# kazuto1011/dusty-gan

Hardware: NVIDIA B200
Metric: chamfer_pairs_per_s (higher is better)
Workload: dtype f32

## Files before the change

dusty-gan_b200/csrc/chamfer.cu:

```cuda
#include <algorithm>

#include "common.cuh"

namespace dusty {
namespace chamfer {

constexpr int TPB = 256;
constexpr int TILE = 2048;
constexpr int CHUNK = 32;

struct Params {
  const float4* scanX;
  const float4* scanY;
  long long strideX, strideY;
  int countX, countY;
  int paddedX, paddedY;
  int row_begin, row_stride;
  int symmetric, mirror, compact_rows;
  float* M;
  long long ldm;
  float* dist1; float* dist2;
  int* idx1; int* idx2;
  const int2* metaX; const int2* metaY;
  const float4* boxX; const float4* boxY;
  const float4* bbX; const float4* bbY;
  const int* permX; const int* permY;
  unsigned long long* visited;
  unsigned long long* keys;
  int n_total, n_ref, offX, offY;
};

template <int NT>
__device__ __forceinline__ double block_sum(double v, double* red) {
  #pragma unroll
  for (int o = 16; o > 0; o >>= 1) v += __shfl_down_sync(0xffffffffu, v, o);
  const int warp = threadIdx.x >> 5, lane = threadIdx.x & 31;
  __syncthreads();
  if (lane == 0) red[warp] = v;
  __syncthreads();
  double s = 0.0;
  if (threadIdx.x == 0) {
    #pragma unroll
    for (int w = 0; w < NT / 32; ++w) s += red[w];
  }
  return s;
}

__device__ __forceinline__ float search_window(float ax, float ay, float az, float cur) {
  const float an = fmaf(az, az, fmaf(ax, ax, ay * ay));
  return fmaf(2.86102295e-6f , an + fmaxf(cur + an, 0.0f), 1e-36f);
}

template <bool WANT_INDEX>
__device__ __forceinline__ void warp_tile_exact_min(const float4* tp, int npairs, float ax, float ay, float az, int lane,
                                                    float& best, int& best_pos) {
  const f32x2 ax2 = pack2(ax, ax), ay2 = pack2(ay, ay), az2 = pack2(az, az);
  float e = __int_as_float(0x7f800000);
  int ei = 0x7fffffff;
  for (int q = lane; q < npairs; q += 32) {
    const float4 q0 = tp[2 * q], q1 = tp[2 * q + 1];
    const f32x2 dx = sub2(pack2(q0.x, q0.y), ax2);
    const f32x2 dy = sub2(pack2(q0.z, q0.w), ay2);
    const f32x2 dz = sub2(pack2(q1.x, q1.y), az2);
    float lo, hi;
    unpack2(fma2(dz, dz, fma2(dx, dx, mul2(dy, dy))), lo, hi);
    if (WANT_INDEX) {
      if (lo < e) { e = lo; ei = 2 * q; }
      if (hi < e) { e = hi; ei = 2 * q + 1; }
    } else {
      e = min3(e, lo, hi);
    }
  }
  float m = e;
  #pragma unroll
  for (int o = 16; o > 0; o >>= 1) m = fminf(m, __shfl_xor_sync(0xffffffffu, m, o));
  best = m;
  if (WANT_INDEX) {
    const bool mine = e == m && ei != 0x7fffffff;
    const unsigned key = mine ? (unsigned)ei : 0x7fffffffu;
    const unsigned kmin = __reduce_min_sync(0xffffffffu, key);
    const unsigned who = __ballot_sync(0xffffffffu, mine && key == kmin);
    best_pos = who ? __shfl_sync(0xffffffffu, ei, __ffs(who) - 1) : 0x7fffffff;
  }
}

template <bool WANT_INDEX>
__device__ __forceinline__ void warp_cloud_exact_min(const float4* cloud, int nchunks, const float4* boxes, float thr,
                                                     float ax, float ay, float az, int lane, const int* perm, float& best,
                                                     int& best_pos) {
  const f32x2 ax2 = pack2(ax, ax), ay2 = pack2(ay, ay), az2 = pack2(az, az);
  float e = __int_as_float(0x7f800000);
  int ei = 0x7fffffff;
  for (int ch = lane; ch < nchunks; ch += 32) {
    if (boxes != nullptr) {
      const float4 bl = boxes[2 * ch], bh = boxes[2 * ch + 1];
      const float gx = max3(0.0f, bl.x - ax, ax - bh.x), gy = max3(0.0f, bl.y - ay, ay - bh.y), gz = max3(0.0f, bl.z - az, az - bh.z);
      if (bl.w == 0.0f && fmaf(gz, gz, fmaf(gx, gx, __fmul_rn(gy, gy))) > thr) continue;
    }
    const float4* cp = cloud + (long long)ch * CHUNK;
    #pragma unroll 4
    for (int k = 0; k < CHUNK / 2; ++k) {
      const float4 q0 = cp[2 * k], q1 = cp[2 * k + 1];
      const f32x2 dx = sub2(pack2(q0.x, q0.y), ax2);
      const f32x2 dy = sub2(pack2(q0.z, q0.w), ay2);
      const f32x2 dz = sub2(pack2(q1.x, q1.y), az2);
      float lo, hi;
      unpack2(fma2(dz, dz, fma2(dx, dx, mul2(dy, dy))), lo, hi);
      if (WANT_INDEX) {
        const int i0 = ch * CHUNK + 2 * k;
        if (lo < e || (lo == e && ei != 0x7fffffff && (perm ? perm[i0] < perm[ei] : i0 < ei))) { e = lo; ei = i0; }
        if (hi < e || (hi == e && ei != 0x7fffffff && (perm ? perm[i0 + 1] < perm[ei] : i0 + 1 < ei))) { e = hi; ei = i0 + 1; }
      } else {
        e = min3(e, lo, hi);
      }
    }
  }
  float m = e;
  #pragma unroll
  for (int o = 16; o > 0; o >>= 1) m = fminf(m, __shfl_xor_sync(0xffffffffu, m, o));
  best = m;
  if (WANT_INDEX) {
    const bool mine = e == m && ei != 0x7fffffff;
    const unsigned key = mine ? (unsigned)(perm ? perm[ei] : ei) : 0x7fffffffu;
    const unsigned kmin = __reduce_min_sync(0xffffffffu, key);
    const unsigned who = __ballot_sync(0xffffffffu, mine && key == kmin);
    best_pos = who ? __shfl_sync(0xffffffffu, ei, __ffs(who) - 1) : 0x7fffffff;
  }
}

__device__ __forceinline__ void emit_entry(const Params& p, int ci, int cj, double S0, double S1) {
  const float v = (float)(S0 / (double)p.countX) + (float)(S1 / (double)p.countY);
  if (p.M) {
    p.M[(long long)(p.compact_rows ? (int)blockIdx.y : ci) * p.ldm + cj] = v;
    if (p.symmetric && p.mirror && ci != cj) p.M[(long long)cj * p.ldm + ci] = v;
  }
  if (p.keys) {
    const int gi = p.offX + ci, gj = p.offY + cj;
    if (gi != gj) {
      const unsigned long long vb = (unsigned long long)__float_as_uint(v) << 32;
      atomicMin(p.keys + gj, vb | (unsigned)gi);
      atomicMin(p.keys + gi, vb | (unsigned)gj);
      const int lo = min(gi, gj), hi = max(gi, gj);
      if (lo < p.n_ref && hi >= p.n_ref) {
        atomicMin(p.keys + p.n_total + hi, vb | (unsigned)lo);
        atomicMin(p.keys + 2 * (long long)p.n_total + lo, vb | (unsigned)hi);
      }
    }
  }
}

template <int R, bool MATRIX, bool MERGED, int NT = TPB>
__global__ void __launch_bounds__(NT, R >= 8 ? 512 / NT : (R == 4 ? 3 : 4)) nn_kernel(const Params p) {
  static_assert(!MERGED || MATRIX, "merged origins are a matrix front end layout");
  extern __shared__ __align__(128) unsigned char smem_raw[];
  float4* const tiles = reinterpret_cast<float4*>(smem_raw);
  __shared__ uint64_t bars[2];
  __shared__ double red[NT / 32];

  constexpr int RB = NT * R;
  constexpr int CH = (NT < TPB && !MERGED) ? CHUNK / 2 : CHUNK;
  constexpr int PR = CH / 2;
  const int tid = threadIdx.x;
  const int lane = tid & 31;

  int ci, cj;
  int dir_only = -1, rb_only = 0;
  if (MATRIX) {
    ci = p.row_begin + blockIdx.y * p.row_stride;
    cj = blockIdx.x;
    if (p.symmetric && cj < ci) return;
  } else {
    ci = cj = blockIdx.y;
    dir_only = blockIdx.z;
    rb_only = blockIdx.x;
    const int rows_here = dir_only == 0 ? p.countX : p.countY;
    if (rb_only >= (rows_here + RB - 1) / RB) return;
  }
  const float4* const sx = p.scanX + (long long)ci * p.strideX;
  const float4* const sy = p.scanY + (long long)cj * p.strideY;

  int2 mx = make_int2(p.countX, 1), my = make_int2(p.countY, 1);
  if (MERGED) { mx = p.metaX[ci]; my = p.metaY[cj]; }
#define K_ROW(r) (MERGED ? rb * RB + (tid >> 5) * (32 * R) + (r) * 32 + lane : rb * RB + (r) * NT + tid)
#define K_countX (MERGED ? mx.x : p.countX)
#define K_countY (MERGED ? my.x : p.countY)
#define K_paddedX (MERGED ? (mx.x + CHUNK - 1) / CHUNK * CHUNK : p.paddedX)
#define K_paddedY (MERGED ? (my.x + CHUNK - 1) / CHUNK * CHUNK : p.paddedY)

  const int ntX = (K_paddedX + TILE - 1) / TILE, ntY = (K_paddedY + TILE - 1) / TILE;
  const int nrbX = (K_countX + RB - 1) / RB, nrbY = (K_countY + RB - 1) / RB;
  const int seg0 = nrbX * ntY;
  int pos_begin, pos_end;
  if (MATRIX) { pos_begin = 0; pos_end = seg0 + nrbY * ntX; }
  else if (dir_only == 0) { pos_begin = rb_only * ntY; pos_end = pos_begin + ntY; }
  else { pos_begin = seg0 + rb_only * ntX; pos_end = pos_begin + ntX; }

  const int tstride = (R >= 8 && NT == TPB) ? TILE : min(TILE, max(p.paddedX, p.paddedY));
  if (tid == 0) { mbar_init(&bars[0], 1); mbar_init(&bars[1], 1); mbar_fence_init(); }
  __syncthreads();

  auto issue = [&](int pos, int buf) {
    int dir, t;
    if (pos < seg0) { dir = 0; t = pos % ntY; } else { dir = 1; t = (pos - seg0) % ntX; }
    const float4* src = (dir == 0 ? sy : sx) + (long long)t * TILE;
    const int padded = dir == 0 ? K_paddedY : K_paddedX;
    const int npts = min(TILE, padded - t * TILE);
    mbar_expect_tx(&bars[buf], (uint32_t)npts * 16u);
    bulk_g2s(tiles + buf * tstride, src, (uint32_t)npts * 16u, &bars[buf]);
  };
  if (tid == 0) issue(pos_begin, 0);

  f32x2 nax[R], nay[R], naz[R];
  float eb[R];
  int ei[R];
  float cur[R], sec[R];
  int cid[R];
// ... 128 lines not shown
        while (flagged) {
          const int src = __ffs(flagged) - 1;
          flagged &= flagged - 1;
          float m;
          int mi = 0;
          warp_tile_exact_min<!MATRIX>(tp, nch * PR, __shfl_sync(0xffffffffu, ax, src), __shfl_sync(0xffffffffu, ay, src),
                                       __shfl_sync(0xffffffffu, az, src), lane, m, mi);
          if (lane == src) {
            if (MATRIX) {
              eb[r] = fminf(eb[r], m);
            } else if (mi != 0x7fffffff) {
              mi += t * TILE;
              if (m < eb[r] || (m == eb[r] && mi < ei[r])) { eb[r] = m; ei[r] = mi; }
            }
          }
        }
      }
    }

    }

    if (MERGED && t == nt - 1 && rb * RB + (tid >> 5) * (32 * R) < rowcount) {
      const float4* const cand = dir == 0 ? sy : sx;
      #pragma unroll
      for (int r = 0; r < R; ++r) {
        float ax, ay, az, dummy;
        unpack2(nax[r], ax, dummy); unpack2(nay[r], ay, dummy); unpack2(naz[r], az, dummy);
        ax *= -0.5f; ay *= -0.5f; az *= -0.5f;
        const bool live = K_ROW(r) < rowcount;
        float e = __int_as_float(0x7f800000);
        if (live && cur[r] < __int_as_float(0x7f800000)) {
          const f32x2 ax2 = pack2(ax, ax), ay2 = pack2(ay, ay), az2 = pack2(az, az);
          const float4* cp = cand + (long long)cid[r] * CHUNK;
          #pragma unroll 4
          for (int k = 0; k < CHUNK / 2; ++k) {
            const float4 q0 = cp[2 * k], q1 = cp[2 * k + 1];
            const f32x2 dx = sub2(pack2(q0.x, q0.y), ax2);
            const f32x2 dy = sub2(pack2(q0.z, q0.w), ay2);
            const f32x2 dz = sub2(pack2(q1.x, q1.y), az2);
            float lo, hi;
            unpack2(fma2(dz, dz, fma2(dx, dx, mul2(dy, dy))), lo, hi);
            e = min3(e, lo, hi);
          }
        }
        eb[r] = e;
        const bool near_tie = live && sec[r] <= cur[r] + search_window(ax, ay, az, cur[r]);
        unsigned flagged = __ballot_sync(0xffffffffu, near_tie);
        while (flagged) {
          const int src = __ffs(flagged) - 1;
          flagged &= flagged - 1;
          float m;
          int mi;
          warp_cloud_exact_min<false>(cand, scanpadded / CHUNK, nullptr, 0.0f, __shfl_sync(0xffffffffu, ax, src),
                                      __shfl_sync(0xffffffffu, ay, src), __shfl_sync(0xffffffffu, az, src), lane, nullptr, m, mi);
          if (lane == src) eb[r] = fminf(eb[r], m);
        }
      }
    }

    if (t == nt - 1) {
      #pragma unroll
      for (int r = 0; r < R; ++r) {
        const int row = K_ROW(r);
        if (row < rowcount) {
          if (MATRIX) {
            if (MERGED) dsum += (row == rowcount - 1 ? (double)(dir == 0 ? mx.y : my.y) : 1.0) * (double)eb[r];
            else dsum += (double)eb[r];
          } else {
            float* dist = dir == 0 ? p.dist1 : p.dist2;
            int* idx = dir == 0 ? p.idx1 : p.idx2;
            const long long o = (long long)ci * rowcount + row;
            dist[o] = eb[r];
            if (idx) idx[o] = ei[r] == 0x7fffffff ? 0 : ei[r];
          }
        }
      }
    }
    if (MATRIX && pos == seg0 - 1) { S0 = block_sum<NT>(dsum, red); dsum = 0.0; }
    __syncthreads();
  }

  if (MATRIX) {
    const double S1 = block_sum<NT>(dsum, red);
    if (tid == 0) emit_entry(p, ci, cj, S0, S1);
  }
}

#undef K_ROW
#undef K_countX
#undef K_countY
#undef K_paddedX
#undef K_paddedY

__global__ void __launch_bounds__(256) prep_kernel(const float* __restrict__ xyz, long long clouds, int count,
                                                   int padded, float4* __restrict__ out) {
  const long long half = padded / 2;
  const long long g = (long long)blockIdx.x * blockDim.x + threadIdx.x;
  if (g >= clouds * half) return;
  const long long c = g / half;
  const int q = (int)(g - c * half);
  const float nan = __int_as_float(0x7fc00000);
  float v[2][4];
  #pragma unroll
  for (int s = 0; s < 2; ++s) {
    const int pt = 2 * q + s;
    if (pt < count) {
      const float* src = xyz + (c * count + pt) * 3;
      const float x = src[0], y = src[1], z = src[2];
      v[s][0] = x; v[s][1] = y; v[s][2] = z;
      v[s][3] = fmaf(z, z, fmaf(x, x, y * y));
    } else {
      v[s][0] = v[s][1] = v[s][2] = v[s][3] = nan;
    }
  }
  out[g * 2] = make_float4(v[0][0], v[1][0], v[0][1], v[1][1]);
  out[g * 2 + 1] = make_float4(v[0][2], v[1][2], v[0][3], v[1][3]);
}

__global__ void __launch_bounds__(256) prep_merge_kernel(const float* __restrict__ xyz, int count, long long stride,
                                                         float4* __restrict__ out, int2* __restrict__ meta) {
  __shared__ int wsum[8];
  const long long c = blockIdx.x;
  const int tid = threadIdx.x, lane = tid & 31, warp = tid >> 5;
  const float* src = xyz + c * count * 3;
  float* dst = reinterpret_cast<float*>(out + c * stride);
  const int per = (count + 255) / 256;
  const int begin = min(tid * per, count), end = min(begin + per, count);
  int mine = 0;
  for (int i = begin; i < end; ++i) mine += (src[3 * i] != 0.0f) || (src[3 * i + 1] != 0.0f) || (src[3 * i + 2] != 0.0f);
  int inc = mine;
  #pragma unroll
  for (int o = 1; o < 32; o <<= 1) { const int t = __shfl_up_sync(0xffffffffu, inc, o); if (lane >= o) inc += t; }
  if (lane == 31) wsum[warp] = inc;
  __syncthreads();
  int before = 0, total = 0;
  #pragma unroll
  for (int w = 0; w < 8; ++w) { if (w < warp) before += wsum[w]; total += wsum[w]; }
  auto put = [&](int pos, float x, float y, float z, float n) {
    float* q = dst + (size_t)(pos >> 1) * 8 + (pos & 1);
    q[0] = x; q[2] = y; q[4] = z; q[6] = n;
  };
  int pos = before + inc - mine;
  for (int i = begin; i < end; ++i) {
    const float x = src[3 * i], y = src[3 * i + 1], z = src[3 * i + 2];
    if (x != 0.0f || y != 0.0f || z != 0.0f) put(pos++, x, y, z, fmaf(z, z, fmaf(x, x, y * y)));
  }
  const int zeros = count - total;
  const int kept = total + (zeros > 0 ? 1 : 0);
  if (tid == 0) {
    if (zeros > 0) put(total, 0.0f, 0.0f, 0.0f, 0.0f);
    meta[c] = make_int2(kept, zeros > 0 ? zeros : 1);
  }
  const float nan = __int_as_float(0x7fc00000);
  const int padded = (kept + CHUNK - 1) / CHUNK * CHUNK;
  for (int i = kept + tid; i < padded; i += 256) put(i, nan, nan, nan, nan);
}

constexpr int SORT_CAP = 32768;
constexpr int SORT_TPB = 1024;
constexpr int WALK_BLOCKS = SORT_CAP / CHUNK / 32;

__device__ __forceinline__ unsigned spread7(unsigned v) {
  v &= 0x7fu;
  v = (v | (v << 4)) & 0x070fu;
  v = (v | (v << 2)) & 0x1333u;
  v = (v | (v << 1)) & 0x1555u;
  return v;
// ... 505 lines not shown
  if (n == 0 || m == 0) {
    if (n) DUSTY_CUDA(cudaMemsetAsync(grad_xyz1, 0, sizeof(float) * 3 * b * n, st));
    if (m) DUSTY_CUDA(cudaMemsetAsync(grad_xyz2, 0, sizeof(float) * 3 * b * m, st));
    return 0;
  }
  if (!xyz1 || !xyz2 || !grad_dist1 || !grad_dist2 || !idx1 || !idx2 || !grad_xyz1 || !grad_xyz2)
    return fail_arg(DUSTY_EINVAL, "chamfer_backward: null pointer");
  const GradArgs a{b, n, m, xyz1, xyz2, grad_dist1, grad_dist2, idx1, idx2, grad_xyz1, grad_xyz2};
  const long long total = (long long)b * n + (long long)b * m;
  const unsigned grid = (unsigned)((total + 255) / 256);
  grad_own_kernel<<<grid, 256, 0, st>>>(a);
  DUSTY_AFTER_LAUNCH("chamfer grad_own_kernel");
  grad_scatter_kernel<<<grid, 256, 0, st>>>(a);
  DUSTY_AFTER_LAUNCH("chamfer grad_scatter_kernel");
  return 0;
}

extern "C" size_t dusty_chamfer_matrix_workspace_bytes(int na, int pa, int nb, int pb) {
  size_t s = 0;
  if (na > 0 && pa > 0) s += align_up(scan_bytes(na, pa), 256) + meta_bytes(na) + box_bytes(na, pa);
  if (nb > 0 && pb > 0) s += align_up(scan_bytes(nb, pb), 256) + meta_bytes(nb) + box_bytes(nb, pb);
  return s;
}

namespace {
struct FusedKeys {
  unsigned long long* keys = nullptr;
  int n_total = 0, n_ref = 0, off_a = 0, off_b = 0;
};
}

static int matrix_impl(const float* A, int na, int pa, const float* B, int nb, int pb, int row_begin, int row_end,
                       int row_stride, int flags, float* M, long long ldm, const FusedKeys& fk, void* workspace,
                       size_t workspace_bytes, void* stream) {
  cudaStream_t st = static_cast<cudaStream_t>(stream);
  const int symmetric = (flags & DUSTY_MATRIX_SYMMETRIC) != 0, mirror = (flags & DUSTY_MATRIX_MIRROR) != 0;
  const int compact_rows = (flags & DUSTY_MATRIX_COMPACT_ROWS) != 0, prepared = (flags & DUSTY_MATRIX_PREPARED) != 0;
  const int merge = (flags & DUSTY_MATRIX_MERGE_ORIGIN) != 0;
  if (mirror && (!symmetric || compact_rows)) return fail_arg(DUSTY_EINVAL, "chamfer_matrix: MIRROR needs SYMMETRIC and excludes COMPACT_ROWS");
  if (na < 0 || nb < 0 || pa <= 0 || pb <= 0) return fail_arg(DUSTY_EINVAL, "chamfer_matrix: bad sizes na=%d pa=%d nb=%d pb=%d", na, pa, nb, pb);
  if (symmetric && (nb != na || pb != pa)) return fail_arg(DUSTY_EINVAL, "chamfer_matrix: symmetric needs nb==na and pb==pa");
  if (row_stride <= 0 || row_begin < 0 || row_end > na || (M && ldm < nb))
    return fail_arg(DUSTY_EINVAL, "chamfer_matrix: bad row range [%d,%d) stride %d of %d, ldm %lld", row_begin, row_end, row_stride, na, ldm);
  if (fk.keys && (fk.n_ref < 0 || fk.off_a < 0 || fk.off_b < 0 || fk.off_a + na > fk.n_total || fk.off_b + nb > fk.n_total ||
                  (symmetric && fk.off_a != fk.off_b)))
    return fail_arg(DUSTY_EINVAL, "chamfer_matrix_fused: offsets %d+%d, %d+%d do not fit %d stacked clouds", fk.off_a, na, fk.off_b, nb, fk.n_total);
  if (row_begin >= row_end || nb == 0) return 0;
  if (int rc = check_device()) return rc;
  if (!A || !B || (!M && !fk.keys) || !workspace) return fail_arg(DUSTY_EINVAL, "chamfer_matrix: null pointer");
  if (!aligned16(workspace)) return fail_arg(DUSTY_EALIGN, "chamfer_matrix: workspace must be 16-byte aligned");
  const size_t need = dusty_chamfer_matrix_workspace_bytes(na, pa, symmetric ? 0 : nb, pb);
  if (workspace_bytes < need) return fail_arg(DUSTY_ENOSPACE, "chamfer_matrix: workspace %zu < %zu", workspace_bytes, need);
  char* const wsp = static_cast<char*>(workspace);
  float4* sa = reinterpret_cast<float4*>(wsp);
  int2* ma = reinterpret_cast<int2*>(wsp + align_up(scan_bytes(na, pa), 256));
  float4* ba = reinterpret_cast<float4*>(wsp + align_up(scan_bytes(na, pa), 256) + meta_bytes(na));
  char* const wsb = wsp + align_up(scan_bytes(na, pa), 256) + meta_bytes(na) + box_bytes(na, pa);
  float4* sb = symmetric ? sa : reinterpret_cast<float4*>(wsb);
  int2* mb = symmetric ? ma : reinterpret_cast<int2*>(wsb + align_up(scan_bytes(nb, pb), 256));
  float4* bb = symmetric ? ba : reinterpret_cast<float4*>(wsb + align_up(scan_bytes(nb, pb), 256) + meta_bytes(nb));
  const bool pair = merge && pa <= PAIR_CAP && pb <= PAIR_CAP;
  const bool walk = merge && !pair && pa <= SORT_CAP && pb <= SORT_CAP;
  const bool sorted = pair || walk;
  if (!prepared) {
    if (sorted) {
      if (int rc = run_prep_sort2(sort_side(A, na, pa, sa, ma, ba, nullptr, nullptr), na,
                                  sort_side(B, nb, pb, sb, mb, bb, nullptr, nullptr), symmetric ? 0 : nb, st, true)) return rc;
    } else if (merge) {
      if (int rc = run_prep_merge(A, na, pa, sa, ma, st)) return rc;
      if (!symmetric) if (int rc = run_prep_merge(B, nb, pb, sb, mb, st)) return rc;
    } else {
      if (int rc = run_prep(A, na, pa, sa, st)) return rc;
      if (!symmetric) if (int rc = run_prep(B, nb, pb, sb, st)) return rc;
    }
  }
  const int rows = (row_end - row_begin + row_stride - 1) / row_stride;
  if (rows > 65535) return fail_arg(DUSTY_EINVAL, "chamfer_matrix: %d rows in one call exceeds 65535", rows);
  Params p{};
  p.scanX = sa; p.scanY = sb;
  p.countX = pa; p.countY = pb;
  p.paddedX = padded_of(pa); p.paddedY = padded_of(pb);
  p.strideX = p.paddedX; p.strideY = p.paddedY;
  p.row_begin = row_begin; p.row_stride = row_stride;
  p.symmetric = symmetric; p.mirror = mirror; p.compact_rows = compact_rows;
  p.M = M; p.ldm = ldm;
  p.keys = fk.keys; p.n_total = fk.n_total; p.n_ref = fk.n_ref; p.offX = fk.off_a; p.offY = fk.off_b;
  p.visited = g_visited_counter;
  const dim3 grid(nb, rows, 1);
  if (merge) {
    p.metaX = ma; p.metaY = mb;
    if (sorted) { p.boxX = ba; p.boxY = bb; p.bbX = block_boxes_of(ba, na, pa); p.bbY = symmetric ? p.bbX : block_boxes_of(bb, nb, pb); }
    if (pair) return launch_pair_split(p, grid, st);
    if (walk) return launch_walk_split<true>(p, grid, st);
    return launch_nn<8, true, true>(p, grid, st);
  }
  return dispatch_matrix(pa > pb ? pa : pb, p, grid, st);
}

extern "C" int dusty_chamfer_matrix(const float* A, int na, int pa, const float* B, int nb, int pb, int row_begin,
                                    int row_end, int row_stride, int flags, float* M, long long ldm, void* workspace,
                                    size_t workspace_bytes, void* stream) {
  if (!M) return fail_arg(DUSTY_EINVAL, "chamfer_matrix: null pointer");
  return matrix_impl(A, na, pa, B, nb, pb, row_begin, row_end, row_stride, flags, M, ldm, FusedKeys{}, workspace,
                     workspace_bytes, stream);
}

extern "C" size_t dusty_nn_keys_bytes(int n_total) { return n_total > 0 ? (size_t)3 * n_total * sizeof(unsigned long long) : 0; }

extern "C" int dusty_nn_keys_reset(uint64_t* keys, int n_total, void* stream) {
  if (n_total <= 0) return 0;
  if (!keys) return fail_arg(DUSTY_EINVAL, "nn_keys_reset: null pointer");
  DUSTY_CUDA(cudaMemsetAsync(keys, 0xff, dusty_nn_keys_bytes(n_total), static_cast<cudaStream_t>(stream)));
  return 0;
}

extern "C" int dusty_chamfer_matrix_fused(const float* A, int na, int pa, const float* B, int nb, int pb, int row_begin,
                                          int row_end, int row_stride, int flags, float* M, long long ldm, int stacked_offset_a,
                                          int stacked_offset_b, int n_ref, int n_total, uint64_t* keys, void* workspace,
                                          size_t workspace_bytes, void* stream) {
  if (!keys) return fail_arg(DUSTY_EINVAL, "chamfer_matrix_fused: null keys");
  FusedKeys fk;
  fk.keys = reinterpret_cast<unsigned long long*>(keys);
  fk.n_total = n_total; fk.n_ref = n_ref; fk.off_a = stacked_offset_a; fk.off_b = stacked_offset_b;
  return matrix_impl(A, na, pa, B, nb, pb, row_begin, row_end, row_stride, flags, M, ldm, fk, workspace, workspace_bytes, stream);
}

extern "C" int dusty_chamfer_count_pairs(int enable, uint64_t* pairs_out) {
  if (pairs_out) {
    *pairs_out = 0;
    if (g_visited_counter) {
      DUSTY_CUDA(cudaDeviceSynchronize());
      unsigned long long v = 0;
      DUSTY_CUDA(cudaMemcpy(&v, g_visited_counter, sizeof(v), cudaMemcpyDeviceToHost));
      *pairs_out = v;
    }
  }
  if (enable && !g_visited_counter) {
    DUSTY_CUDA(cudaMalloc(&g_visited_counter, sizeof(unsigned long long)));
  }
  if (g_visited_counter) DUSTY_CUDA(cudaMemset(g_visited_counter, 0, sizeof(unsigned long long)));
  if (!enable && g_visited_counter) { DUSTY_CUDA(cudaFree(g_visited_counter)); g_visited_counter = nullptr; }
  return 0;
}
```

dusty-gan_b200/csrc/chamfer_pair.cuh:

```cuda
constexpr int PAIR_CAP = 2048;
constexpr int PAIR_NW = 8;

__global__ void __launch_bounds__(PAIR_NW * 32, 3) nn_pair_split_kernel(const Params p) {
  constexpr int SUB = 8;
  constexpr int GR = 32;
  extern __shared__ __align__(128) unsigned char smem_raw[];
  __shared__ uint64_t bar;
  __shared__ double tsum[2 * (PAIR_CAP / GR)];
  __shared__ int next_task;
  const int tid = threadIdx.x, lane = tid & 31;
  const int h = lane >> 4, l16 = lane & 15;

  const int ci = p.row_begin + blockIdx.y * p.row_stride;
  const int cj = blockIdx.x;
  if (p.symmetric && cj < ci) return;

  const int2 mx = p.metaX[ci], my = p.metaY[cj];
  const int padX = (mx.x + CHUNK - 1) / CHUNK * CHUNK, padY = (my.x + CHUNK - 1) / CHUNK * CHUNK;
  float4* const sX = reinterpret_cast<float4*>(smem_raw);
  float4* const sY = sX + p.paddedX;
  float4* const bX = sY + p.paddedY;
  float4* const bY = bX + p.paddedX / CHUNK * 2;
  if (tid == 0) {
    mbar_init(&bar, 1);
    mbar_fence_init();
    next_task = 0;
    const uint32_t bytes = (uint32_t)(padX + padY) * 16u + (uint32_t)(padX / CHUNK + padY / CHUNK) * 32u;
    mbar_expect_tx(&bar, bytes);
    bulk_g2s(sX, p.scanX + (long long)ci * p.strideX, (uint32_t)padX * 16u, &bar);
    bulk_g2s(sY, p.scanY + (long long)cj * p.strideY, (uint32_t)padY * 16u, &bar);
    bulk_g2s(bX, p.boxX + (long long)ci * (p.paddedX / CHUNK * 2), (uint32_t)(padX / CHUNK) * 32u, &bar);
    bulk_g2s(bY, p.boxY + (long long)cj * (p.paddedY / CHUNK * 2), (uint32_t)(padY / CHUNK) * 32u, &bar);
  }
  __syncthreads();
  mbar_wait(&bar, 0);

  const int ngX = (mx.x + GR - 1) / GR, ngY = (my.x + GR - 1) / GR;
  const float inf = __int_as_float(0x7f800000);

  for (;;) {
    int task = 0;
    if (lane == 0) task = atomicAdd(&next_task, 1);
    task = __shfl_sync(0xffffffffu, task, 0);
    if (task >= ngX + ngY) break;
    const int dir = task >= ngX;
    const int g = dir ? task - ngX : task;
    const float4* const rows = dir ? sY : sX;
    const float4* const cand = dir ? sX : sY;
    const float4* const rbox = dir ? bY : bX;
    const float4* const cbox = dir ? bX : bY;
    const int rowcount = dir ? my.x : mx.x;
    const int nch = (dir ? padX : padY) / CHUNK;

    f32x2 nax[2], nay[2], naz[2];
    float cur[2], sec[2];
    int cid[2];
    float rx[2], ry[2], rz[2];
    #pragma unroll
    for (int j = 0; j < 2; ++j) {
      const int row = g * GR + j * 16 + l16;
      const int rr = row < rowcount ? row : 0;
      const float* f = reinterpret_cast<const float*>(rows + (rr >> 1) * 2) + (rr & 1);
      rx[j] = f[0]; ry[j] = f[2]; rz[j] = f[4];
      const float mx2 = -2.0f * rx[j], my2 = -2.0f * ry[j], mz2 = -2.0f * rz[j];
      nax[j] = pack2(mx2, mx2); nay[j] = pack2(my2, my2); naz[j] = pack2(mz2, mz2);
      cur[j] = sec[j] = inf; cid[j] = 0;
    }
    const float oax = h ? rx[1] : rx[0], oay = h ? ry[1] : ry[0], oaz = h ? rz[1] : rz[0];
    const float an = fmaf(oaz, oaz, fmaf(oax, oax, oay * oay));
    const int orow = g * GR + lane;
    float ubr = orow < rowcount ? inf : -1.0f;
    float gl0, gl1, gl2, gh0, gh1, gh2;
    {
      const float4 bl = rbox[2 * g], bh = rbox[2 * g + 1];
      gl0 = bl.x; gl1 = bl.y; gl2 = bl.z; gh0 = bh.x; gh1 = bh.y; gh2 = bh.z;
      if (bl.w != 0.0f) {
        gl0 = fminf(gl0, 0.0f); gl1 = fminf(gl1, 0.0f); gl2 = fminf(gl2, 0.0f);
        gh0 = fmaxf(gh0, 0.0f); gh1 = fmaxf(gh1, 0.0f); gh2 = fmaxf(gh2, 0.0f);
      }
    }
    const bool forced = cbox[2 * (nch - 1)].w != 0.0f;
    unsigned key[2];
    #pragma unroll
    for (int q = 0; q < 2; ++q) {
      const int c = q * 32 + lane;
      key[q] = 0xffffffffu;
      if (forced && c == nch - 1) {
        key[q] = (unsigned)c;
      } else if (c < nch) {
        const float4 bl = cbox[2 * c], bh = cbox[2 * c + 1];
        const float gx = max3(0.0f, bl.x - gh0, gl0 - bh.x), gy = max3(0.0f, bl.y - gh1, gl1 - bh.y), gz = max3(0.0f, bl.z - gh2, gl2 - bh.z);
        const float lb = fmaf(gz, gz, fmaf(gx, gx, __fmul_rn(gy, gy)));
        if (lb < inf) key[q] = (__float_as_uint(lb) & ~63u) | (unsigned)c;
      }
    }
    float ubmax = inf;
    int nvis = 0;
    for (;;) {
      const unsigned kwin = __reduce_min_sync(0xffffffffu, min(key[0], key[1]));
      if (kwin == 0xffffffffu) break;
      if (__uint_as_float(kwin & ~63u) > ubmax) break;
      const int c = (int)(kwin & 63u);
      if (key[0] == kwin) key[0] = 0xffffffffu;
      if (key[1] == kwin) key[1] = 0xffffffffu;
      const float4 bl = cbox[2 * c], bh = cbox[2 * c + 1];
      const float qx = max3(0.0f, bl.x - oax, oax - bh.x), qy = max3(0.0f, bl.y - oay, oay - bh.y), qz = max3(0.0f, bl.z - oaz, oaz - bh.z);
      const bool need = (forced && c == nch - 1) || fmaf(qz, qz, fmaf(qx, qx, __fmul_rn(qy, qy))) <= ubr;
      if (!__any_sync(0xffffffffu, need)) continue;
      ++nvis;
      const float4* cp = cand + c * CHUNK + h * (CHUNK / 2);
      #pragma unroll
      for (int w = 0; w < 2; ++w) {
        float cm[2];
        #pragma unroll
        for (int k = w * 4; k < w * 4 + 4; ++k) {
          const float4 q0 = cp[2 * k], q1 = cp[2 * k + 1];
          const f32x2 bx = pack2(q0.x, q0.y), by = pack2(q0.z, q0.w);
          const f32x2 bz = pack2(q1.x, q1.y), bn = pack2(q1.z, q1.w);
          #pragma unroll
          for (int j = 0; j < 2; ++j) {
            f32x2 s = fma2(naz[j], bz, bn);
            s = fma2(nay[j], by, s);
            s = fma2(nax[j], bx, s);
            float lo, hi;
            unpack2(s, lo, hi);
            cm[j] = (k == w * 4) ? fminf(lo, hi) : min3(cm[j], lo, hi);
          }
        }
        const int wid = c * (CHUNK / SUB) + 2 * h + w;
        #pragma unroll
        for (int j = 0; j < 2; ++j) {
          const bool better = cm[j] < cur[j];
          sec[j] = fminf(sec[j], better ? cur[j] : cm[j]);
          cur[j] = fminf(cur[j], cm[j]);
          cid[j] = better ? wid : cid[j];
        }
      }
      const float other = __shfl_xor_sync(0xffffffffu, h ? cur[0] : cur[1], 16);
      if (ubr >= 0.0f) {
        const float dest = fmaxf(fminf(h ? cur[1] : cur[0], other) + an, 0.0f);
        ubr = fmaf(3.81469727e-6f , an + dest, dest) + 1e-36f;
      }
      ubmax = __uint_as_float(__reduce_max_sync(0xffffffffu, __float_as_uint(fmaxf(ubr, 0.0f))));
    }
    if (p.visited != nullptr && lane == 0)
      atomicAdd(p.visited, (unsigned long long)nvis * CHUNK * (unsigned long long)min(GR, rowcount - g * GR));

    const float pc = __shfl_xor_sync(0xffffffffu, h ? cur[0] : cur[1], 16);
    const float ps = __shfl_xor_sync(0xffffffffu, h ? sec[0] : sec[1], 16);
    const int pi = __shfl_xor_sync(0xffffffffu, h ? cid[0] : cid[1], 16);
    const float mc = h ? cur[1] : cur[0], ms = h ? sec[1] : sec[0];
    const int mi0 = h ? cid[1] : cid[0];
    const bool theirs = pc < mc;
    const float c1 = fminf(mc, pc);
    const float s1 = fminf(fminf(ms, ps), theirs ? mc : pc);
    const int w1 = theirs ? pi : mi0;
    const bool live = orow < rowcount;
    float e = inf;
    if (live && c1 < inf) {
      const f32x2 ax2 = pack2(oax, oax), ay2 = pack2(oay, oay), az2 = pack2(oaz, oaz);
      const float4* cp = cand + w1 * SUB;
      #pragma unroll
      for (int k = 0; k < SUB / 2; ++k) {
        const int kk = (k + lane) & (SUB / 2 - 1);
        const float4 q0 = cp[2 * kk], q1 = cp[2 * kk + 1];
        const f32x2 dx = sub2(pack2(q0.x, q0.y), ax2);
        const f32x2 dy = sub2(pack2(q0.z, q0.w), ay2);
        const f32x2 dz = sub2(pack2(q1.x, q1.y), az2);
        float lo, hi;
        unpack2(fma2(dz, dz, fma2(dx, dx, mul2(dy, dy))), lo, hi);
        e = min3(e, lo, hi);
      }
    }
    const bool near_tie = live && s1 <= c1 + search_window(oax, oay, oaz, c1);
    unsigned flagged = __ballot_sync(0xffffffffu, near_tie);
    while (flagged) {
      const int src = __ffs(flagged) - 1;
      flagged &= flagged - 1;
      float m;
      int mi;
      warp_cloud_exact_min<false>(cand, nch, cbox, __shfl_sync(0xffffffffu, e, src), __shfl_sync(0xffffffffu, oax, src),
                                  __shfl_sync(0xffffffffu, oay, src), __shfl_sync(0xffffffffu, oaz, src), lane, nullptr, m, mi);
      if (lane == src) e = fminf(e, m);
    }
    double dsum = live ? (orow == rowcount - 1 ? (double)(dir ? my.y : mx.y) : 1.0) * (double)e : 0.0;
    #pragma unroll
    for (int o = 16; o > 0; o >>= 1) dsum += __shfl_down_sync(0xffffffffu, dsum, o);
    if (lane == 0) tsum[task] = dsum;
  }

  __syncthreads();
  if (tid == 0) {
    double S0 = 0.0, S1 = 0.0;
    for (int t = 0; t < ngX; ++t) S0 += tsum[t];
    for (int t = ngX; t < ngX + ngY; ++t) S1 += tsum[t];
    emit_entry(p, ci, cj, S0, S1);
  }
}

static int launch_pair_split(const Params& p, dim3 grid, cudaStream_t st) {
  const size_t smem = (size_t)(p.paddedX + p.paddedY) * 16 + (size_t)(p.paddedX / CHUNK + p.paddedY / CHUNK) * 32;
  static bool configured[kMaxDevices] = {};
  const int dev = current_device();
  if (!configured[dev]) {
    DUSTY_CUDA(cudaFuncSetAttribute(nn_pair_split_kernel, cudaFuncAttributeMaxDynamicSharedMemorySize,
                                    2 * PAIR_CAP * 16 + 2 * (PAIR_CAP / CHUNK) * 32));
    configured[dev] = true;
  }
  nn_pair_split_kernel<<<grid, PAIR_NW * 32, smem, st>>>(p);
  DUSTY_AFTER_LAUNCH("chamfer nn_pair_split_kernel");
  return 0;
}
```

dusty-gan_b200/csrc/chamfer_walk.cuh:

```cuda
constexpr int WALK_NW = 8;
constexpr int WALK_TPC = 8;
constexpr int WALK_SPLIT_MAXTASKS = 2 * (SORT_CAP / 32 + 1);

template <bool MATRIX>
__global__ void __launch_bounds__(WALK_NW * 32, 3) nn_walk_split_kernel(const Params p) {
  constexpr int SUB = 8;
  constexpr int GR = 32;
  __shared__ double tsum[MATRIX ? WALK_SPLIT_MAXTASKS : 1];
  __shared__ int next_task;
  __shared__ float4 stage[WALK_NW][CHUNK];
  const int tid = threadIdx.x, lane = tid & 31;
  const int h = lane >> 4, l16 = lane & 15;
  int ci, cj;
  if (MATRIX) {
    ci = p.row_begin + blockIdx.y * p.row_stride;
    cj = blockIdx.x;
    if (p.symmetric && cj < ci) return;
  } else {
    ci = cj = blockIdx.y;
  }
  const int2 mx = p.metaX[ci], my = p.metaY[cj];
  const int padX = (mx.x + CHUNK - 1) / CHUNK * CHUNK, padY = (my.x + CHUNK - 1) / CHUNK * CHUNK;
  const float4* const sX = p.scanX + (long long)ci * p.strideX;
  const float4* const sY = p.scanY + (long long)cj * p.strideY;
// ... 114 lines not shown
            sec[j] = fminf(sec[j], better ? cur[j] : cm[j]);
            cur[j] = fminf(cur[j], cm[j]);
            cid[j] = better ? wid : cid[j];
          }
        }
        const float other = __shfl_xor_sync(0xffffffffu, h ? cur[0] : cur[1], 16);
        if (ubr >= 0.0f) {
          const float dest = fmaxf(fminf(h ? cur[1] : cur[0], other) + an, 0.0f);
          ubr = fmaf(3.81469727e-6f , an + dest, dest) + 1e-36f;
        }
        ubmax = __uint_as_float(__reduce_max_sync(0xffffffffu, __float_as_uint(fmaxf(ubr, 0.0f))));
      }
    }
    if (p.visited != nullptr && lane == 0)
      atomicAdd(p.visited, (unsigned long long)nvis * CHUNK * (unsigned long long)min(GR, rowcount - g * GR));

    const float pc = __shfl_xor_sync(0xffffffffu, h ? cur[0] : cur[1], 16);
    const float ps = __shfl_xor_sync(0xffffffffu, h ? sec[0] : sec[1], 16);
    const int pi = __shfl_xor_sync(0xffffffffu, h ? cid[0] : cid[1], 16);
    const float mc = h ? cur[1] : cur[0], ms = h ? sec[1] : sec[0];
    const int mi0 = h ? cid[1] : cid[0];
    const bool theirs = pc < mc;
    const float c1 = fminf(mc, pc);
    const float s1 = fminf(fminf(ms, ps), theirs ? mc : pc);
    const int w1 = theirs ? pi : mi0;
    const bool live = orow < rowcount;
    float e = inf;
    int eidx = 0x7fffffff;
    if (live && c1 < inf) {
      const f32x2 ax2 = pack2(oax, oax), ay2 = pack2(oay, oay), az2 = pack2(oaz, oaz);
      const float4* cp = cand + (long long)w1 * SUB;
      #pragma unroll
      for (int k = 0; k < SUB / 2; ++k) {
        const float4 q0 = __ldg(cp + 2 * k), q1 = __ldg(cp + 2 * k + 1);
        const f32x2 dx = sub2(pack2(q0.x, q0.y), ax2);
        const f32x2 dy = sub2(pack2(q0.z, q0.w), ay2);
        const f32x2 dz = sub2(pack2(q1.x, q1.y), az2);
        float lo, hi;
        unpack2(fma2(dz, dz, fma2(dx, dx, mul2(dy, dy))), lo, hi);
        if (MATRIX) {
          e = min3(e, lo, hi);
        } else {
          const int i0 = w1 * SUB + 2 * k;
          if (lo < e || (lo == e && eidx != 0x7fffffff && cperm[i0] < cperm[eidx])) { e = lo; eidx = i0; }
          if (hi < e || (hi == e && eidx != 0x7fffffff && cperm[i0 + 1] < cperm[eidx])) { e = hi; eidx = i0 + 1; }
        }
      }
    }
    const bool near_tie = live && s1 <= c1 + search_window(oax, oay, oaz, c1);
    unsigned flagged = __ballot_sync(0xffffffffu, near_tie);
    while (flagged) {
      const int src = __ffs(flagged) - 1;
      flagged &= flagged - 1;
      float m;
      int mi = 0x7fffffff;
      warp_cloud_exact_min<!MATRIX>(cand, nch, cbox, __shfl_sync(0xffffffffu, e, src), __shfl_sync(0xffffffffu, oax, src),
                                    __shfl_sync(0xffffffffu, oay, src), __shfl_sync(0xffffffffu, oaz, src), lane, cperm, m, mi);
      if (lane == src) {
        if (MATRIX) {
          e = fminf(e, m);
        } else if (mi != 0x7fffffff && (m < e || (m == e && (eidx == 0x7fffffff || cperm[mi] < cperm[eidx])))) {
          e = m; eidx = mi;
        }
      }
    }
    if (MATRIX) {
      double dsum = live ? (orow == rowcount - 1 ? (double)(dir ? my.y : mx.y) : 1.0) * (double)e : 0.0;
      #pragma unroll
      for (int o = 16; o > 0; o >>= 1) dsum += __shfl_down_sync(0xffffffffu, dsum, o);
      if (lane == 0) tsum[task] = dsum;
    } else if (live) {
      const long long o = (long long)ci * (dir ? p.strideY : p.strideX) + orow;
      (dir ? p.dist2 : p.dist1)[o] = e;
      (dir ? p.idx2 : p.idx1)[o] = cperm[eidx == 0x7fffffff ? 0 : eidx];
    }
  }

  if (MATRIX) {
    __syncthreads();
    if (tid == 0) {
      double S0 = 0.0, S1 = 0.0;
      for (int t = 0; t < ngX; ++t) S0 += tsum[t];
      for (int t = ngX; t < ngX + ngY; ++t) S1 += tsum[t];
      emit_entry(p, ci, cj, S0, S1);
    }
  }
}

template <bool MATRIX>
static int launch_walk_split(const Params& p, dim3 grid, cudaStream_t st) {
  nn_walk_split_kernel<MATRIX><<<grid, WALK_NW * 32, 0, st>>>(p);
  DUSTY_AFTER_LAUNCH("chamfer nn_walk_split_kernel");
  return 0;
}
```

dusty-gan_b200/csrc/common.cuh:

```cuda
#pragma once

#include <cuda_runtime.h>
#include <stdint.h>
#include <stddef.h>

#include "dusty_b200.h"

namespace dusty {

int fail_cuda(cudaError_t e, const char* what);
int fail_arg(int code, const char* fmt, ...);
void count_launches(int n);
int check_device();
int current_device();
constexpr int kMaxDevices = 64;

constexpr int kNumSMs = 148;

inline size_t align_up(size_t v, size_t a) { return (v + a - 1) / a * a; }
inline bool aligned16(const void* p) { return (reinterpret_cast<uintptr_t>(p) & 15u) == 0; }

#define DUSTY_CUDA(call)                                                    \
  do {                                                                      \
    cudaError_t e__ = (call);                                               \
    if (e__ != cudaSuccess) return ::dusty::fail_cuda(e__, #call);          \
  } while (0)

#define DUSTY_AFTER_LAUNCH(name)                                            \
  do {                                                                      \
    ::dusty::count_launches(1);                                             \
    cudaError_t e__ = cudaGetLastError();                                   \
    if (e__ != cudaSuccess) return ::dusty::fail_cuda(e__, name);           \
  } while (0)

#ifdef __CUDACC__

typedef unsigned long long f32x2;

__device__ __forceinline__ f32x2 pack2(float lo, float hi) {
  f32x2 r; asm("mov.b64 %0, {%1, %2};" : "=l"(r) : "f"(lo), "f"(hi)); return r;
}
__device__ __forceinline__ void unpack2(f32x2 v, float& lo, float& hi) {
  asm("mov.b64 {%0, %1}, %2;" : "=f"(lo), "=f"(hi) : "l"(v));
}
__device__ __forceinline__ f32x2 fma2(f32x2 a, f32x2 b, f32x2 c) {
  f32x2 d; asm("fma.rn.f32x2 %0, %1, %2, %3;" : "=l"(d) : "l"(a), "l"(b), "l"(c)); return d;
}
__device__ __forceinline__ f32x2 mul2(f32x2 a, f32x2 b) {
  f32x2 d; asm("mul.rn.f32x2 %0, %1, %2;" : "=l"(d) : "l"(a), "l"(b)); return d;
}
__device__ __forceinline__ f32x2 sub2(f32x2 a, f32x2 b) {
  f32x2 d; asm("sub.rn.f32x2 %0, %1, %2;" : "=l"(d) : "l"(a), "l"(b)); return d;
}
__device__ __forceinline__ float min3(float a, float b, float c) {
  float d; asm("min.f32 %0, %1, %2, %3;" : "=f"(d) : "f"(a), "f"(b), "f"(c)); return d;
}
__device__ __forceinline__ float max3(float a, float b, float c) {
  float d; asm("max.f32 %0, %1, %2, %3;" : "=f"(d) : "f"(a), "f"(b), "f"(c)); return d;
}

__device__ __forceinline__ uint32_t smem_u32(const void* p) {
  return static_cast<uint32_t>(__cvta_generic_to_shared(p));
}
__device__ __forceinline__ void mbar_init(uint64_t* bar, uint32_t count) {
  asm volatile("mbarrier.init.shared::cta.b64 [%0], %1;" ::"r"(smem_u32(bar)), "r"(count) : "memory");
}
__device__ __forceinline__ void mbar_fence_init() {
  asm volatile("fence.mbarrier_init.release.cluster;" ::: "memory");
}
__device__ __forceinline__ void mbar_expect_tx(uint64_t* bar, uint32_t bytes) {
  asm volatile("mbarrier.arrive.expect_tx.shared::cta.b64 _, [%0], %1;" ::"r"(smem_u32(bar)), "r"(bytes) : "memory");
}
__device__ __forceinline__ void mbar_wait(uint64_t* bar, uint32_t parity) {
  asm volatile(
      "{\n\t"
      ".reg .pred p;\n\t"
      "WAIT_%=:\n\t"
      "mbarrier.try_wait.parity.shared::cta.b64 p, [%0], %1;\n\t"
      "@p bra DONE_%=;\n\t"
      "bra WAIT_%=;\n\t"
      "DONE_%=:\n\t"
      "}" ::"r"(smem_u32(bar)), "r"(parity) : "memory");
}
__device__ __forceinline__ void bulk_g2s(void* smem_dst, const void* gmem_src, uint32_t bytes, uint64_t* bar) {
  asm volatile("cp.async.bulk.shared::cluster.global.mbarrier::complete_tx::bytes [%0], [%1], %2, [%3];" ::"r"(
                   smem_u32(smem_dst)),
               "l"(gmem_src), "r"(bytes), "r"(smem_u32(bar))
               : "memory");
}

__device__ __forceinline__ float4 ldg_stream(const float4* p) {
  float4 r;
  asm volatile("ld.global.nc.L1::no_allocate.v4.f32 {%0,%1,%2,%3}, [%4];"
               : "=f"(r.x), "=f"(r.y), "=f"(r.z), "=f"(r.w) : "l"(p));
  return r;
}
__device__ __forceinline__ void stg_stream(float4* p, const float4& v) {
  asm volatile("st.global.L1::no_allocate.v4.f32 [%0], {%1,%2,%3,%4};" ::"l"(p), "f"(v.x), "f"(v.y), "f"(v.z), "f"(v.w) : "memory");
}

#endif

}
```

Measured before the change: 7.655 million.

## Make pair-split chamfer kernel persistent with triple-buffered TMA prefetch of cloud pairs

The pair-split kernel now runs as a persistent grid sized to SM occupancy. Each CTA walks (row, col) cells in a grid-stride order, skipping dead symmetric cells. Each CTA holds three shared-memory slots, and bulk async copies prefetch upcoming cloud pairs while 24 warps dynamically pull tasks from the current slot. The last warp to finish a cell reduces its sums, refills that slot and emits the entry. The aim is to hide load latency and per-CTA launch and setup cost across pairs, at the price of one large CTA per SM and more complex cross-warp synchronization with volatile shared state.

```diff
diff --git a/dusty-gan_b200/csrc/chamfer.cu b/dusty-gan_b200/csrc/chamfer.cu
--- a/dusty-gan_b200/csrc/chamfer.cu
+++ b/dusty-gan_b200/csrc/chamfer.cu
@@ -16,6 +16,7 @@
   int countX, countY;
   int paddedX, paddedY;
   int row_begin, row_stride;
+  int rows, cols;
   int symmetric, mirror, compact_rows;
   float* M;
   long long ldm;
@@ -128,10 +129,10 @@
   }
 }
 
-__device__ __forceinline__ void emit_entry(const Params& p, int ci, int cj, double S0, double S1) {
+__device__ __forceinline__ void emit_entry(const Params& p, int ci, int cj, int row, double S0, double S1) {
   const float v = (float)(S0 / (double)p.countX) + (float)(S1 / (double)p.countY);
   if (p.M) {
-    p.M[(long long)(p.compact_rows ? (int)blockIdx.y : ci) * p.ldm + cj] = v;
+    p.M[(long long)(p.compact_rows ? row : ci) * p.ldm + cj] = v;
     if (p.symmetric && p.mirror && ci != cj) p.M[(long long)cj * p.ldm + ci] = v;
   }
   if (p.keys) {
@@ -426,7 +427,7 @@
 
   if (MATRIX) {
     const double S1 = block_sum<NT>(dsum, red);
-    if (tid == 0) emit_entry(p, ci, cj, S0, S1);
+    if (tid == 0) emit_entry(p, ci, cj, blockIdx.y, S0, S1);
   }
 }
 
@@ -1098,6 +1099,7 @@
   p.paddedX = padded_of(pa); p.paddedY = padded_of(pb);
   p.strideX = p.paddedX; p.strideY = p.paddedY;
   p.row_begin = row_begin; p.row_stride = row_stride;
+  p.rows = rows; p.cols = nb;
   p.symmetric = symmetric; p.mirror = mirror; p.compact_rows = compact_rows;
   p.M = M; p.ldm = ldm;
   p.keys = fk.keys; p.n_total = fk.n_total; p.n_ref = fk.n_ref; p.offX = fk.off_a; p.offY = fk.off_b;
@@ -1106,7 +1108,7 @@
   if (merge) {
     p.metaX = ma; p.metaY = mb;
     if (sorted) { p.boxX = ba; p.boxY = bb; p.bbX = block_boxes_of(ba, na, pa); p.bbY = symmetric ? p.bbX : block_boxes_of(bb, nb, pb); }
-    if (pair) return launch_pair_split(p, grid, st);
+    if (pair) return launch_pair_split(p, st);
     if (walk) return launch_walk_split<true>(p, grid, st);
     return launch_nn<8, true, true>(p, grid, st);
   }
diff --git a/dusty-gan_b200/csrc/chamfer_pair.cuh b/dusty-gan_b200/csrc/chamfer_pair.cuh
--- a/dusty-gan_b200/csrc/chamfer_pair.cuh
+++ b/dusty-gan_b200/csrc/chamfer_pair.cuh
@@ -1,48 +1,117 @@
 constexpr int PAIR_CAP = 2048;
-constexpr int PAIR_NW = 8;
-
-__global__ void __launch_bounds__(PAIR_NW * 32, 3) nn_pair_split_kernel(const Params p) {
+constexpr int PAIR_NW = 24;
+constexpr int PAIR_SLOTS = 3;
+constexpr int PAIR_MAXTASKS = 2 * (PAIR_CAP / 32);
+
+__device__ __forceinline__ void pair_skip_dead(const Params& p, int& r, int& c) {
+  while (r < p.rows && p.symmetric && c < p.row_begin + r * p.row_stride) {
+    c += gridDim.x;
+    r += c / p.cols;
+    c %= p.cols;
+  }
+}
+__device__ __forceinline__ void pair_next(const Params& p, int& r, int& c) {
+  c += gridDim.x;
+  r += c / p.cols;
+  c %= p.cols;
+  pair_skip_dead(p, r, c);
+}
+
+__global__ void __launch_bounds__(PAIR_NW * 32, 1) nn_pair_split_kernel(const Params p) {
   constexpr int SUB = 8;
   constexpr int GR = 32;
   extern __shared__ __align__(128) unsigned char smem_raw[];
-  __shared__ uint64_t bar;
-  __shared__ double tsum[2 * (PAIR_CAP / GR)];
-  __shared__ int next_task;
+  __shared__ uint64_t bar[PAIR_SLOTS];
+  __shared__ double tsum[PAIR_SLOTS][PAIR_MAXTASKS];
+  __shared__ int next_task[PAIR_SLOTS], left[PAIR_SLOTS];
+  __shared__ int4 meta[PAIR_SLOTS];
+  __shared__ int2 cell[PAIR_SLOTS];
+  __shared__ int warp_seq[PAIR_NW];
   const int tid = threadIdx.x, lane = tid & 31;
   const int h = lane >> 4, l16 = lane & 15;
-
-  const int ci = p.row_begin + blockIdx.y * p.row_stride;
-  const int cj = blockIdx.x;
-  if (p.symmetric && cj < ci) return;
-
-  const int2 mx = p.metaX[ci], my = p.metaY[cj];
-  const int padX = (mx.x + CHUNK - 1) / CHUNK * CHUNK, padY = (my.x + CHUNK - 1) / CHUNK * CHUNK;
-  float4* const sX = reinterpret_cast<float4*>(smem_raw);
-  float4* const sY = sX + p.paddedX;
-  float4* const bX = sY + p.paddedY;
-  float4* const bY = bX + p.paddedX / CHUNK * 2;
+  const size_t slot_bytes = (size_t)(p.paddedX + p.paddedY) * 16 + (size_t)(p.paddedX / CHUNK + p.paddedY / CHUNK) * 32;
+  const auto slot_of = [&](int s) { return reinterpret_cast<float4*>(smem_raw + s * slot_bytes); };
+
+  const auto fill = [&](int s, int r, int c) {
+    const int ci = p.row_begin + r * p.row_stride;
+    const int2 mx = p.metaX[ci], my = p.metaY[c];
+    const int padX = (mx.x + CHUNK - 1) / CHUNK * CHUNK, padY = (my.x + CHUNK - 1) / CHUNK * CHUNK;
+    float4* const sX = slot_of(s);
+    float4* const sY = sX + p.paddedX;
+    float4* const bX = sY + p.paddedY;
+    float4* const bY = bX + p.paddedX / CHUNK * 2;
+    meta[s] = make_int4(mx.x, mx.y, my.x, my.y);
+    cell[s] = make_int2(r, c);
+    next_task[s] = 0;
+    left[s] = 0;
+    fence_proxy_async_smem();
+    const uint32_t bytes = (uint32_t)(padX + padY) * 16u + (uint32_t)(padX / CHUNK + padY / CHUNK) * 32u;
+    mbar_expect_tx(&bar[s], bytes);
+    bulk_g2s(sX, p.scanX + (long long)ci * p.strideX, (uint32_t)padX * 16u, &bar[s]);
+    bulk_g2s(sY, p.scanY + (long long)c * p.strideY, (uint32_t)padY * 16u, &bar[s]);
+    bulk_g2s(bX, p.boxX + (long long)ci * (p.paddedX / CHUNK * 2), (uint32_t)(padX / CHUNK) * 32u, &bar[s]);
+    bulk_g2s(bY, p.boxY + (long long)c * (p.paddedY / CHUNK * 2), (uint32_t)(padY / CHUNK) * 32u, &bar[s]);
+  };
+
+  int r = blockIdx.x / p.cols, c = blockIdx.x % p.cols;
+  pair_skip_dead(p, r, c);
   if (tid == 0) {
-    mbar_init(&bar, 1);
+    for (int s = 0; s < PAIR_SLOTS; ++s) mbar_init(&bar[s], 1);
     mbar_fence_init();
-    next_task = 0;
-    const uint32_t bytes = (uint32_t)(padX + padY) * 16u + (uint32_t)(padX / CHUNK + padY / CHUNK) * 32u;
-    mbar_expect_tx(&bar, bytes);
-    bulk_g2s(sX, p.scanX + (long long)ci * p.strideX, (uint32_t)padX * 16u, &bar);
-    bulk_g2s(sY, p.scanY + (long long)cj * p.strideY, (uint32_t)padY * 16u, &bar);
-    bulk_g2s(bX, p.boxX + (long long)ci * (p.paddedX / CHUNK * 2), (uint32_t)(padX / CHUNK) * 32u, &bar);
-    bulk_g2s(bY, p.boxY + (long long)cj * (p.paddedY / CHUNK * 2), (uint32_t)(padY / CHUNK) * 32u, &bar);
+    int fr = r, fc = c;
+    for (int s = 0; s < PAIR_SLOTS && fr < p.rows; ++s) {
+      fill(s, fr, fc);
+      pair_next(p, fr, fc);
+    }
   }
   __syncthreads();
-  mbar_wait(&bar, 0);
-
-  const int ngX = (mx.x + GR - 1) / GR, ngY = (my.x + GR - 1) / GR;
+  if (r >= p.rows) return;
+
   const float inf = __int_as_float(0x7f800000);
+  const int warp = tid >> 5;
+  if (lane == 0) warp_seq[warp] = 0;
+  __syncwarp();
+  mbar_wait(&bar[0], 0);
 
   for (;;) {
+    const int seq = *reinterpret_cast<volatile int*>(&warp_seq[warp]);
+    const int s = seq % PAIR_SLOTS;
     int task = 0;
-    if (lane == 0) task = atomicAdd(&next_task, 1);
+    if (lane == 0) task = atomicAdd(&next_task[s], 1);
     task = __shfl_sync(0xffffffffu, task, 0);
-    if (task >= ngX + ngY) break;
+    const volatile int* const m = &meta[s].x;
+    const int2 mx = make_int2(m[0], m[1]), my = make_int2(m[2], m[3]);
+    const int padX = (mx.x + CHUNK - 1) / CHUNK * CHUNK, padY = (my.x + CHUNK - 1) / CHUNK * CHUNK;
+    const int ngX = (mx.x + GR - 1) / GR, ngY = (my.x + GR - 1) / GR;
+    const float4* const sX = slot_of(s);
+    const float4* const sY = sX + p.paddedX;
+    const float4* const bX = sY + p.paddedY;
+    const float4* const bY = bX + p.paddedX / CHUNK * 2;
+    if (task >= ngX + ngY) {
+      int2 rc = cell[s];
+      __syncwarp();
+      int last = 0;
+      if (lane == 0) {
+        __threadfence_block();
+        last = atomicAdd(&left[s], 1) == PAIR_NW - 1;
+        __threadfence_block();
+      }
+      if (last) {
+        double S0 = 0.0, S1 = 0.0;
+        for (int t = 0; t < ngX; ++t) S0 += tsum[s][t];
+        for (int t = ngX; t < ngX + ngY; ++t) S1 += tsum[s][t];
+        int fr = rc.x, fc = rc.y;
+        for (int k = 0; k < PAIR_SLOTS; ++k) pair_next(p, fr, fc);
+        if (fr < p.rows) fill(s, fr, fc);
+        emit_entry(p, p.row_begin + rc.x * p.row_stride, rc.y, rc.x, S0, S1);
+      }
+      pair_next(p, rc.x, rc.y);
+      if (rc.x >= p.rows) break;
+      if (lane == 0) warp_seq[warp] = seq + 1;
+      __syncwarp();
+      mbar_wait(&bar[(seq + 1) % PAIR_SLOTS], (uint32_t)((seq + 1) / PAIR_SLOTS) & 1u);
+      continue;
+    }
     const int dir = task >= ngX;
     const int g = dir ? task - ngX : task;
     const float4* const rows = dir ? sY : sX;
@@ -186,28 +255,26 @@
     double dsum = live ? (orow == rowcount - 1 ? (double)(dir ? my.y : mx.y) : 1.0) * (double)e : 0.0;
     #pragma unroll
     for (int o = 16; o > 0; o >>= 1) dsum += __shfl_down_sync(0xffffffffu, dsum, o);
-    if (lane == 0) tsum[task] = dsum;
-  }
-
-  __syncthreads();
-  if (tid == 0) {
-    double S0 = 0.0, S1 = 0.0;
-    for (int t = 0; t < ngX; ++t) S0 += tsum[t];
-    for (int t = ngX; t < ngX + ngY; ++t) S1 += tsum[t];
-    emit_entry(p, ci, cj, S0, S1);
-  }
-}
-
-static int launch_pair_split(const Params& p, dim3 grid, cudaStream_t st) {
-  const size_t smem = (size_t)(p.paddedX + p.paddedY) * 16 + (size_t)(p.paddedX / CHUNK + p.paddedY / CHUNK) * 32;
-  static bool configured[kMaxDevices] = {};
+    if (lane == 0) tsum[*reinterpret_cast<volatile int*>(&warp_seq[warp]) % PAIR_SLOTS][task] = dsum;
+  }
+}
+
+static int launch_pair_split(const Params& p, cudaStream_t st) {
+  const size_t slot = (size_t)(p.paddedX + p.paddedY) * 16 + (size_t)(p.paddedX / CHUNK + p.paddedY / CHUNK) * 32;
+  static int ctas[kMaxDevices] = {};
   const int dev = current_device();
-  if (!configured[dev]) {
-    DUSTY_CUDA(cudaFuncSetAttribute(nn_pair_split_kernel, cudaFuncAttributeMaxDynamicSharedMemorySize,
-                                    2 * PAIR_CAP * 16 + 2 * (PAIR_CAP / CHUNK) * 32));
-    configured[dev] = true;
-  }
-  nn_pair_split_kernel<<<grid, PAIR_NW * 32, smem, st>>>(p);
+  if (!ctas[dev]) {
+    const int max_smem = PAIR_SLOTS * (2 * PAIR_CAP * 16 + 2 * (PAIR_CAP / CHUNK) * 32);
+    DUSTY_CUDA(cudaFuncSetAttribute(nn_pair_split_kernel, cudaFuncAttributeMaxDynamicSharedMemorySize, max_smem));
+    int sms = 0, per_sm = 0;
+    DUSTY_CUDA(cudaDeviceGetAttribute(&sms, cudaDevAttrMultiProcessorCount, dev));
+    DUSTY_CUDA(cudaOccupancyMaxActiveBlocksPerMultiprocessor(&per_sm, nn_pair_split_kernel, PAIR_NW * 32, max_smem));
+    ctas[dev] = sms * per_sm;
+  }
+  long long live = (long long)p.rows * p.cols;
+  if (p.symmetric) live -= (long long)p.rows * p.row_begin + (long long)p.row_stride * p.rows * (p.rows - 1) / 2;
+  const int grid = (int)std::min<long long>(ctas[dev], live);
+  nn_pair_split_kernel<<<grid, PAIR_NW * 32, PAIR_SLOTS * slot, st>>>(p);
   DUSTY_AFTER_LAUNCH("chamfer nn_pair_split_kernel");
   return 0;
 }
diff --git a/dusty-gan_b200/csrc/chamfer_walk.cuh b/dusty-gan_b200/csrc/chamfer_walk.cuh
--- a/dusty-gan_b200/csrc/chamfer_walk.cuh
+++ b/dusty-gan_b200/csrc/chamfer_walk.cuh
@@ -220,7 +220,7 @@
       double S0 = 0.0, S1 = 0.0;
       for (int t = 0; t < ngX; ++t) S0 += tsum[t];
       for (int t = ngX; t < ngX + ngY; ++t) S1 += tsum[t];
-      emit_entry(p, ci, cj, S0, S1);
+      emit_entry(p, ci, cj, blockIdx.y, S0, S1);
     }
   }
 }
diff --git a/dusty-gan_b200/csrc/common.cuh b/dusty-gan_b200/csrc/common.cuh
--- a/dusty-gan_b200/csrc/common.cuh
+++ b/dusty-gan_b200/csrc/common.cuh
@@ -88,6 +88,9 @@
                "l"(gmem_src), "r"(bytes), "r"(smem_u32(bar))
                : "memory");
 }
+__device__ __forceinline__ void fence_proxy_async_smem() {
+  asm volatile("fence.proxy.async.shared::cta;" ::: "memory");
+}
 
 __device__ __forceinline__ float4 ldg_stream(const float4* p) {
   float4 r;
```

Result: slower. 7.431 million, median of 6 (-2.9%).
